# twosigma/Cook

Hardware: AMD Instinct MI355X
Metric: match-cycles/sec at 1M pending x 50k offers (higher is better)
Workload: dtype f64

## Files before the change

cook_amd/csrc/classfit_asm.hpp:

```cpp
#pragma once
#if CF_SLOTS_N == 12
#define CF_O_CTRL "13728"
#define CF_O_CTRL4 "13732"
#define CF_O_ARR "15280"
#define CF_O_CLS32 "9504"
#define CF_SLOT_SHIFT "9"
#define CF_SLOT_N "12"
#define CF_ROW_END "3072"
#elif CF_SLOTS_N == 24
#define CF_O_CTRL "16800"
#define CF_O_CTRL4 "16804"
#define CF_O_ARR "18352"
#define CF_O_CLS32 "12576"
#define CF_SLOT_SHIFT "10"
#define CF_SLOT_N "24"
#define CF_ROW_END "6144"
#else
#error "CF_SLOTS_N: 12 or 24"
#endif
#ifndef CF_ASM_WAIT_READS
#define CF_ASM_WAIT_READS "30"
#endif
#ifdef CF_DELAY_D
#define CF_ASM_DELAY_D "s_sleep 6\n\t"
#else
#define CF_ASM_DELAY_D
#endif
#define CF_ASM_DECIDER_RUN \
   \
  "v_lshl_add_u32 v114, v65, 3, s56\n\t" \
  "ds_read_b64 v[114:115], v114\n\t" \
  "s_ff1_i32_b64 s44, s[42:43]\n\t" \
  "s_lshl_b32 s45, s44, 12\n\t" \
  "s_add_u32 s45, s45, s59\n\t" \
  "s_lshl_b32 s47, s57, 8\n\t" \
  "s_or_b32 s47, s47, s44\n\t" \
  "s_mov_b32 s41, 1\n\t"  \
   \
  "0:\n\t" \
  "v_readlane_b32 s60, v80, s44\n\t" \
  "v_readlane_b32 s61, v81, s44\n\t" \
  "v_readlane_b32 s62, v82, s44\n\t" \
  "s_and_b32 s63, s62, 0xffff00ff\n\t"  \
  "s_cmp_lg_u32 s63, 0\n\t" \
  "s_cbranch_scc1 9f\n\t" \
                                                                                           \
  "v_mov_b32_e32 v88, s47\n\t"                                                                                                          \
  "v_add_u32_e32 v100, s46, v83\n\t"                                                                                                    \
  "s_mov_b64 exec, 1\n\t"                                                                                                               \
  "ds_write_b32 v87, v88 offset:" CF_O_CTRL4 "\n\t"                                                                                              \
  "s_mov_b64 exec, -1\n\t"                                                                                                              \
  "s_mov_b32 s82, " CF_ASM_WAIT_READS "\n\t"              \
  "1:\n\t"                                                                                                                              \
  "ds_read_b32 v92, v100\n\t"                                                                                                           \
  "ds_read_b64 v[94:95], v100 offset:8\n\t"                                                                                             \
  "ds_read_b128 v[96:99], v100 offset:16\n\t"                                                                                           \
  "ds_read_b32 v93, v100\n\t"                                                                                                           \
                                        \
  "v_subrev_u32_e32 v101, s60, v71\n\t"                                                                                                 \
  "v_subrev_u32_e32 v102, s61, v72\n\t"                                                                                                 \
  "v_cvt_f64_u32_e32 v[104:105], v101\n\t"                                                                                              \
  "v_cvt_f64_u32_e32 v[106:107], v102\n\t"                                                                                              \
  "v_mul_f64 v[104:105], v[104:105], v[66:67]\n\t"                                                                                      \
  "v_mul_f64 v[106:107], v[106:107], v[68:69]\n\t"                                                                                      \
  "v_add_f64 v[104:105], v[104:105], v[106:107]\n\t"                                                                                    \
  "v_add_f64 v[104:105], -v[104:105], 1.0\n\t"                                                                                          \
  "v_cmp_le_u32_e64 s[64:65], s60, v71\n\t"                                                                                             \
  "v_cmp_le_u32_e64 s[66:67], s61, v72\n\t"                                                                                             \
  "v_cmp_ne_u32_e64 s[68:69], 0, v64\n\t"                                                                                               \
  "s_and_b64 s[64:65], s[64:65], s[66:67]\n\t"                                                                                          \
  "s_and_b64 s[64:65], s[64:65], s[68:69]\n\t"                                                                                          \
  "s_waitcnt lgkmcnt(0)\n\t"                                                                                                            \
        \
  "s_bfe_u32 s63, s62, 0x4000c\n\t"                                                                                                     \
  "s_cmp_eq_u32 s63, 0\n\t"                                                                                                             \
  "s_cbranch_scc1 3f\n\t"                                                                                                               \
  "v_readlane_b32 s66, v85, s44\n\t"                                                                                                    \
  "v_readlane_b32 s67, v86, s44\n\t"                                                                                                    \
  "s_cmp_lt_u32 s63, 1\n\t"                                                                                                           \
  "s_cbranch_scc1 3f\n\t"                                                                                                               \
  "s_bfe_u32 s72, s66, 0x100000\n\t"                                                                      \
  "s_lshr_b32 s73, s72, 8\n\t"                                                                                                          \
  "s_lshl_b32 s73, s73, 3\n\t"                                                                                                          \
  "s_and_b32 s72, s72, 0xff\n\t"                                                                                                        \
  "v_lshrrev_b64 v[108:109], s73, v[114:115]\n\t"                                                                                       \
  "v_and_b32_e32 v108, 0xff, v108\n\t"                                                                                                  \
  "v_cmp_eq_u32_e64 s[74:75], s72, v108\n\t"                                                                                            \
  "s_and_b64 s[64:65], s[64:65], s[74:75]\n\t"                                                                                          \
  "s_cmp_lt_u32 s63, 2\n\t"                                                                                                           \
  "s_cbranch_scc1 3f\n\t"                                                                                                               \
// ... 15 lines not shown
  "v_and_b32_e32 v108, 0xff, v108\n\t"                                                                                                  \
  "v_cmp_eq_u32_e64 s[74:75], s72, v108\n\t"                                                                                            \
  "s_and_b64 s[64:65], s[64:65], s[74:75]\n\t"                                                                                          \
  "s_cmp_lt_u32 s63, 4\n\t"                                                                                                           \
  "s_cbranch_scc1 3f\n\t"                                                                                                               \
  "s_bfe_u32 s72, s67, 0x100010\n\t"                                                                      \
  "s_lshr_b32 s73, s72, 8\n\t"                                                                                                          \
  "s_lshl_b32 s73, s73, 3\n\t"                                                                                                          \
  "s_and_b32 s72, s72, 0xff\n\t"                                                                                                        \
  "v_lshrrev_b64 v[108:109], s73, v[114:115]\n\t"                                                                                       \
  "v_and_b32_e32 v108, 0xff, v108\n\t"                                                                                                  \
  "v_cmp_eq_u32_e64 s[74:75], s72, v108\n\t"                                                                                            \
  "s_and_b64 s[64:65], s[64:65], s[74:75]\n\t"                                                                                          \
  "3:\n\t"                                                                                                                              \
   \
  "v_and_b32_e32 v108, 0xffffff00, v92\n\t"                                                                                             \
  "v_cmp_eq_u32_e64 s[70:71], s45, v108\n\t"                                                                                            \
  "v_cmp_eq_u32_e64 s[72:73], v92, v93\n\t"                                                                                             \
  "v_sub_u32_e32 v108, v73, v92\n\t"                                                                                                    \
  "v_and_b32_e32 v108, 0xff, v108\n\t"                                                                                                  \
  "v_cmp_gt_u32_e64 s[74:75], 3, v108\n\t"                                                                                              \
  "v_and_b32_e32 v109, 0xffff, v94\n\t"                                                                                                 \
  "v_cmp_ne_u32_e64 s[76:77], v109, v74\n\t"                                                                                            \
  "v_cmp_ne_u32_e64 s[78:79], v109, v75\n\t"                                                                                            \
  "v_cmp_gt_i32_e64 s[80:81], 0, v95\n\t"                                                                                               \
  "s_and_b64 s[74:75], s[74:75], s[76:77]\n\t"                                                                                          \
  "s_and_b64 s[74:75], s[74:75], s[78:79]\n\t"                                                                                          \
  "s_or_b64 s[74:75], s[74:75], s[80:81]\n\t"                                                                                           \
  "s_and_b64 s[72:73], s[70:71], s[72:73]\n\t"                                          \
  "s_and_b64 s[70:71], s[72:73], s[74:75]\n\t"                                                                                            \
  "s_andn2_b64 s[76:77], s[52:53], s[70:71]\n\t"                                                                     \
  "s_cmp_eq_u64 s[76:77], 0\n\t"                                                                                                          \
  "s_cbranch_scc1 2f\n\t"                                                                                                                 \
   \
   \
  "s_and_b64 s[78:79], s[76:77], s[72:73]\n\t"                                                                                            \
  "s_cmp_eq_u64 s[78:79], 0\n\t"                                                                                                          \
  "s_cbranch_scc1 4f\n\t"                                                                                                                 \
  "v_and_b32_e32 v109, 0x3fff, v95\n\t"                                                                                                   \
  "s_and_b64 s[72:73], s[64:65], s[54:55]\n\t"                                                   \
  "10:\n\t"                                                                                                                               \
  "s_ff1_i32_b64 s83, s[78:79]\n\t"                                                                                                       \
  "v_readlane_b32 s63, v109, s83\n\t"                                                                                                     \
  "s_bitset0_b64 s[78:79], s83\n\t"                                                                                                       \
  "v_cmp_eq_u32_e64 vcc, s63, v65\n\t"                                                                                                    \
  "s_and_b64 vcc, vcc, s[72:73]\n\t"                                                                                                      \
  "s_cmp_eq_u64 vcc, 0\n\t"                                                                                                               \
  "s_cbranch_scc1 11f\n\t"                                                                                                                \
  "s_bitset1_b64 s[80:81], s83\n\t"                                                                                                       \
  "s_bitset0_b64 s[76:77], s83\n\t"                                                                                                       \
  "11:\n\t"                                                                                                                               \
  "s_cmp_lg_u64 s[78:79], 0\n\t"                                                                                                          \
  "s_cbranch_scc1 10b\n\t"                                                                                                                \
  "s_cmp_eq_u64 s[76:77], 0\n\t"                                                                                                          \
  "s_cbranch_scc1 2f\n\t"                                                                                                                 \
  "4:\n\t"                                                                                                                                \
  "s_sub_u32 s82, s82, 1\n\t"      \
  "s_cmp_eq_u32 s82, 0\n\t"                                                                                                             \
  "s_cbranch_scc1 9f\n\t"                                                                                                               \
  "s_sleep 1\n\t"                                                                                                                       \
  "s_branch 1b\n\t"                                                                                                                     \
  "2:\n\t"                                                                                                                              \
  "s_andn2_b64 s[74:75], s[52:53], s[80:81]\n\t"                                                                        \
  "s_or_b64 s[64:65], s[64:65], s[74:75]\n\t"                                                          \
  "v_cndmask_b32_e64 v110, v98, v104, s[54:55]\n\t"                                                                                     \
  "v_cndmask_b32_e64 v111, v99, v105, s[54:55]\n\t"                                                                                     \
  "v_cndmask_b32_e64 v110, 0, v110, s[64:65]\n\t"                                                                                       \
  "v_cndmask_b32_e64 v111, 0, v111, s[64:65]\n\t"                                                                                       \
  "v_cvt_f32_f64_e32 v112, v[110:111]\n\t" \
   \
   \
   \
  "s_mov_b64 s[84:85], s[42:43]\n\t" \
  "v_mov_b32_e32 v113, v112\n\t" \
  "s_bitset0_b64 s[84:85], s44\n\t" \
// ... 5 lines not shown
  "s_cmp_eq_u32 s46, " CF_ROW_END "\n\t" \
  "s_cselect_b32 s46, 0, s46\n\t" \
  "v_max_f32_dpp v113, v113, v113 row_half_mirror row_mask:0xf bank_mask:0xf\n\t" \
  "s_lshl_b32 s62, s62, 8\n\t" \
  "s_or_b32 s47, s62, s86\n\t" \
  "v_max_f32_dpp v113, v113, v113 row_mirror row_mask:0xf bank_mask:0xf\n\t" \
  "s_lshl_b32 s63, s86, 12\n\t" \
  "s_add_u32 s45, s59, s63\n\t" \
  "v_max_f32_dpp v113, v113, v113 row_bcast:15 row_mask:0xa bank_mask:0xf\n\t" \
  "v_add_f32_e32 v108, 0x35000000, v112\n\t" \
  "v_and_b32_e32 v109, 0x40000000, v95\n\t" \
  "v_max_f32_dpp v113, v113, v113 row_bcast:31 row_mask:0xc bank_mask:0xf\n\t" \
  "v_cmp_ne_u32_e64 s[70:71], 0, v109\n\t" \
  "s_nop 0\n\t" \
  "v_readlane_b32 s63, v113, 63\n\t" \
  "s_cmp_eq_u32 s63, 0\n\t" \
  "s_cbranch_scc1 8f\n\t"  \
  "v_cmp_eq_f32_e64 s[78:79], s63, v112\n\t" \
  "v_cmp_le_f32_e64 s[76:77], s63, v108\n\t"  \
  "s_and_b64 s[76:77], s[76:77], s[64:65]\n\t"                                      \
  "s_bcnt1_i32_b64 s62, s[76:77]\n\t"                                                                                                   \
  "s_cmp_gt_u32 s62, 1\n\t"                                                                                                             \
  "s_cbranch_scc1 9f\n\t"                                                                                                               \
  "s_and_b64 s[70:71], s[70:71], s[76:77]\n\t"                                                                                          \
  "s_and_b64 s[70:71], s[70:71], s[74:75]\n\t"                       \
  "s_cmp_lg_u64 s[70:71], 0\n\t"                                                                                                        \
  "s_cbranch_scc1 9f\n\t"                                                                                                               \
  "s_ff1_i32_b64 s82, s[78:79]\n\t"                                                                                                     \
  "s_cmp_lt_u32 s82, 58\n\t"                                                                                                            \
  "s_cbranch_scc0 5f\n\t"                                                                                                               \
                                                                                                         \
  "v_readlane_b32 s64, v71, s82\n\t"                                                                                                    \
  "v_readlane_b32 s65, v72, s82\n\t"                                                                                                    \
  "v_readlane_b32 s66, v65, s82\n\t"                                                                                                    \
  "s_sub_u32 s67, s64, s60\n\t"                                                                                                         \
  "s_sub_u32 s70, s65, s61\n\t"                                                                                                         \
  "v_cmp_eq_u32_e64 vcc, s82, v84\n\t"                                                                                                  \
  "v_mov_b32_e32 v88, s67\n\t"                                                                                                          \
  "v_mov_b32_e32 v89, s70\n\t"                                                                                                          \
  "s_cmp_lt_u32 s67, s49\n\t" \
  "s_cselect_b32 s71, 1, 0\n\t" \
  "s_cmp_lt_u32 s70, s50\n\t" \
  "s_cselect_b32 s71, 1, s71\n\t" \
  "v_cndmask_b32_e32 v71, v71, v88, vcc\n\t"                                                                                            \
  "v_cndmask_b32_e32 v72, v72, v89, vcc\n\t"                                                                                            \
  "s_cmp_lg_u32 s71, 0\n\t"                                                                                                             \
  "s_cselect_b64 s[62:63], vcc, 0\n\t"                             \
  "s_mov_b32 s72, s44\n\t"                                                                                                              \
  "s_mov_b32 s73, 0\n\t"                                                                                                                \
  "v_cndmask_b32_e64 v64, v64, 0, s[62:63]\n\t"                                                                                         \
  "s_branch 7f\n\t"                                                                                                                     \
        \
  "5:\n\t"                                                                                                                              \
  "v_readlane_b32 s64, v96, s82\n\t"                                                                                                    \
  "v_readlane_b32 s65, v97, s82\n\t"                                                                                                    \
  "v_readlane_b32 s76, v95, s82\n\t"                                                                                                    \
  "v_readlane_b32 s77, v94, s82\n\t"                                                                                                    \
  "v_readlane_b32 s78, v73, s82\n\t"                                                                                                    \
  "s_sub_u32 s67, s64, s60\n\t"                                                                                                         \
  "s_sub_u32 s70, s65, s61\n\t"                                                                                                         \
  "s_and_b32 s66, s76, 0x3fff\n\t"                                                                                                      \
  "s_bfe_u32 s79, s76, 0x80010\n\t"                                                                                                     \
  "s_and_b32 s73, s77, 0xffff\n\t"                                                                                                      \
  "s_lshr_b32 s81, s77, 16\n\t"                                                                                                         \
  "s_sub_u32 s80, s82, 57\n\t"                                                                                                          \
  "s_cmp_lt_u32 s67, s49\n\t" \
// ... 16 lines not shown
  "v_mov_b32_e32 v100, s78\n\t"                                                                                                         \
  "s_mov_b64 exec, 1\n\t"                                                                                                               \
  "ds_write_b64 v90, v[88:89] offset:" CF_O_ARR "\n\t"                                                                                         \
  "ds_write_b32 v91, v100 offset:" CF_O_CTRL4 "\n\t"                                                                                             \
  "s_mov_b64 exec, -1\n\t"                                                                                                              \
  "v_cmp_eq_u32_e64 vcc, s82, v84\n\t"                                                                                                  \
  "v_mov_b32_e32 v101, s73\n\t" \
  "s_lshl_b32 s62, s80, 8\n\t" \
  "v_cndmask_b32_e32 v75, v75, v74, vcc\n\t" \
  "v_cndmask_b32_e32 v74, v74, v101, vcc\n\t" \
  "v_cndmask_b32_e32 v73, v73, v100, vcc\n\t" \
  "s_lshl_b32 s63, s81, 12\n\t"                                                                                                         \
  "s_or_b32 s72, s44, s62\n\t"                                                                                                          \
  "s_or_b32 s72, s72, s63\n\t"                                                                                                          \
  "s_cmp_lg_u32 s71, 0\n\t"                                                                                                             \
  "s_cbranch_scc1 7f\n\t"                                                                              \
  "s_mul_i32 s62, s79, 56\n\t" \
  "v_add_u32_e32 v90, s62, v87\n\t" \
  "ds_read_b128 v[116:119], v90 offset:" CF_O_CLS32 "\n\t"  \
  "v_mov_b32_e32 v88, s66\n\t" \
  "v_lshl_add_u32 v102, v88, 3, s56\n\t"   \
  "ds_read_b64 v[102:103], v102\n\t"                                                                                        \
  "s_andn2_b64 s[62:63], s[54:55], s[68:69]\n\t"                                                                                        \
  "s_ff1_i32_b64 s83, s[62:63]\n\t"                                                                                                     \
  "v_cmp_eq_u32_e64 vcc, s83, v84\n\t"                                                                                                  \
  "v_mov_b32_e32 v89, s79\n\t"                                                                                                          \
  "v_mov_b32_e32 v91, s67\n\t"                                                                                                          \
  "v_mov_b32_e32 v101, s70\n\t"                                                                                                         \
  "v_cndmask_b32_e64 v64, v64, 1, vcc\n\t"                                                                                              \
  "v_cndmask_b32_e32 v65, v65, v88, vcc\n\t"                                                                                            \
  "v_cndmask_b32_e32 v70, v70, v89, vcc\n\t"                                                                                            \
  "v_cndmask_b32_e32 v71, v71, v91, vcc\n\t"                                                                                            \
  "v_cndmask_b32_e32 v72, v72, v101, vcc\n\t"                                                                                           \
  "s_waitcnt lgkmcnt(0)\n\t"                                                                                                            \
  "v_cndmask_b32_e32 v66, v66, v116, vcc\n\t"                                                                                           \
  "v_cndmask_b32_e32 v67, v67, v117, vcc\n\t"                                                                                           \
  "v_cndmask_b32_e32 v68, v68, v118, vcc\n\t"                                                                                           \
  "v_cndmask_b32_e32 v69, v69, v119, vcc\n\t"  \
  "v_cndmask_b32_e32 v114, v114, v102, vcc\n\t" \
  "v_cndmask_b32_e32 v115, v115, v103, vcc\n\t"                                                                                           \
   \
  "7:\n\t"                                                                                                                              \
  "v_cmp_eq_u32_e64 vcc, s44, v84\n\t"                                                                                                  \
  "v_mov_b32_e32 v88, s66\n\t"                                                                                                          \
  "v_cmp_lt_u32_e64 s[62:63], s67, v80\n\t"                                                                                             \
  "v_cmp_lt_u32_e64 s[76:77], s70, v81\n\t"                                                                                             \
  "v_cndmask_b32_e32 v76, v76, v88, vcc\n\t"                                                                                            \
  "s_or_b64 s[62:63], s[62:63], s[76:77]\n\t"                                                                                           \
  "s_lshl_b64 s[76:77], -2, s44\n\t"                                                                                                    \
  "s_and_b64 s[62:63], s[62:63], s[76:77]\n\t"                                                                                          \
  "s_or_b64 s[38:39], s[38:39], s[62:63]\n\t"                                                                                           \
  "s_min_u32 s37, s37, s67\n\t"                                                                                                         \
  "s_min_u32 s40, s40, s70\n\t"                                                                                                         \
  "s_add_u32 s36, s36, 1\n\t"                                                                                                           \
  "v_mov_b32_e32 v88, s72\n\t"                                                                                                          \
  "v_mov_b32_e32 v89, s73\n\t"                                                                                                          \
  "v_mov_b32_e32 v90, s64\n\t"                                                                                                          \
  "v_mov_b32_e32 v91, s65\n\t" \
  "s_mov_b64 exec, 1\n\t" \
  "ds_write_b128 v77, v[88:91]\n\t" \
  "s_mov_b64 exec, -1\n\t" \
  "v_add_u32_e32 v77, 32, v77\n\t"  \
   \
  "8:\n\t" \
  CF_ASM_DELAY_D \
  "s_mov_b64 s[42:43], s[84:85]\n\t" \
  "s_mov_b32 s44, s86\n\t" \
  "s_add_u32 s57, s57, 1\n\t" \
  "s_cmp_lg_u64 s[42:43], 0\n\t" \
  "s_cbranch_scc1 0b\n\t" \
  "s_mov_b32 s41, 0\n\t" \
  "9:\n\t" \
  "s_waitcnt lgkmcnt(0)\n\t"

#define CF_ASM_CLASS_STEP                                                                                                               \
  "v_mov_b32_e32 v80, s44\n\t"                                                                                                          \
  "s_lshl_b32 s60, s45, 2\n\t"                                                                                                          \
  "s_add_u32 s60, s60, s44\n\t"                                                                                                         \
  "v_mov_b32_e32 v81, s60\n\t"                                                                                                          \
  "ds_read_b64 v[82:83], v80 offset:" CF_O_CTRL "\n\t"                                                                     \
  "ds_read_b32 v84, v81 offset:" CF_O_CTRL4 "\n\t"                                                                   \
  "s_mov_b32 s41, 3\n\t"                                                                                                                \
  "s_waitcnt lgkmcnt(0)\n\t"                                                                                                            \
  "v_readfirstlane_b32 s61, v82\n\t"                                                                                                    \
  "v_readfirstlane_b32 s42, v83\n\t"                                                                                                    \
  "v_readfirstlane_b32 s43, v84\n\t"                                                                                                    \
  "s_cmp_lg_u32 s61, 0\n\t"                                                                                                             \
  "s_cbranch_scc1 9f\n\t"                                                                                                               \
// ... 141 lines not shown
```

cook_amd/csrc/classfit_host.hpp:

```cpp

static int classfit_env() {
  static const int v = [] {
    const char* s = std::getenv("COOK_CLASSFIT");
    return s && (s[0] == '0' || s[0] == '1') ? s[0] - '0' : -1;
  }();
  return v;
}
static bool classfit_by_default(const cook_engine* e) {
  const int f = classfit_env();
  if (f >= 0) return f == 1;
  return g_engines_on_device[e->device & 63].load() >= 6;
}
static size_t cf_lds_bytes_host(unsigned NP, unsigned M, bool eq, unsigned G, unsigned S) {
  size_t n = sizeof(CfFixed) + (size_t)NP * 10u;
  n = (n + 7u) & ~(size_t)7u;
  if (eq) n += (size_t)M * 8u;
  n += ((size_t)G + 1u) * 2u + (size_t)G * 2u + (size_t)S * 2u;
  return n + 64u;
}
bool cf_setup(cook_engine* e, const MatchIn& in, const MatchIn* in_dev, const MatchState& st, const JobRec* jr, const JobCons* jcons, const OfferA* oa, const OfferB* ob,
              CfPoolCtx& ctx) {
  const unsigned K = in.K, M = in.M, G = in.G;
  e->cf_inelig = 0x10000u;
  if (K == 0 || M == 0 || M > CF_SORT_N || G > CF_MAXG || in.good_enough < 1.0 || in.has_x || in.reserved_bits || in.host_dup) return false;
// ... 24 lines not shown
  const unsigned NP = (M + 63u) & ~63u;
  const unsigned S = hc.any_group ? e->cf_group_run_total + hc.n_grouped : 0u;
  if (cf_lds_bytes_host(NP, M, hc.any_eq != 0u, hc.any_group ? G : 0u, S) > CF_LDS_BYTES || S > 60000u) {
    e->cf_inelig = CF_X_SHAPE;
    return false;
  }
  ctx.in = in_dev;
  ctx.st = st;
  ctx.b = b;
  return true;
}
static void cf_prof_print(const uint32_t* q) {
#ifdef CF_PROF
  std::fprintf(stderr, "CFPROF (x16 shader cycles) decider: slow steps %u (candidates %u evaluation %u commit %u) plain steps %u in %u walk-total %u | class wave 1: poll %u answer %u answers %u idle %u idles %u | class wave 2: poll %u answer %u answers %u idle %u idles %u | walk ticks(100MHz) %u | batch boundaries: decider %u, batches without a walked job %u\n", q[27], q[24], q[25], q[26], q[28], q[29], q[31], q[32], q[33], q[35], q[36], q[37], q[40], q[41], q[43], q[44], q[45], q[CFS_TICKS_WALK], q[30], q[38]);
  std::fprintf(stderr, "CFPROF plain steps %u, C++ steps %u; steps that left the plain form: gpu kind %u, novel hosts %u, group %u, answer missing after the re-reads %u, guard band %u, epoch end %u\n", q[46], q[47], q[34] & 65535u, q[34] >> 16, q[39] & 65535u, q[39] >> 16, q[42] & 65535u, q[42] >> 16);
#else
  (void)q;
#endif
}
void cf_run(cook_engine* lead, cook_engine* const* es, unsigned n, hipStream_t stream) {
  cook_engine* e = lead;
  for (unsigned i0 = 0; i0 < n; i0 += (unsigned)CF_PACK) {
    const unsigned c = std::min<unsigned>(CF_PACK, n - i0);
    CfPack pk{};
    for (unsigned x = 0; x < (unsigned)CF_PACK; ++x) pk.c[x] = es[i0 + (x < c ? x : 0u)]->placement.walk;
    KLS("cf_walk", stream, cf_walk, c, CF_THREADS, pk);
  }
  for (unsigned i = 0; i < n; ++i) {
    const CfPoolCtx& c = es[i]->placement.walk;
    const unsigned G = es[i]->last_in.G;
// ... 23 lines not shown
```

cook_amd/csrc/classfit_walk.hpp:

```cpp
#pragma once
#if defined(CF_PROF) && !defined(CF_STATS)
#define CF_STATS 1
#endif
#ifdef CF_STATS
#define CF_STAT(x) x
#define CF_TICKS() cook_ticks()
#else
#define CF_STAT(x) ((void)0)
#define CF_TICKS() 0ull
#endif
#ifdef CF_PROF
#define CF_PROF_T(x) const unsigned long long x = __builtin_readcyclecounter()
#define CF_PROF_ADD(i, d) prof[i] += (unsigned long long)(d)
#define CF_PROF_WHY(n) why = why == 3u ? (n) : why
#define CF_PROF_LEAVE() (why < 4u ? leave_a += 1ull << (16u * why) : leave_b += 1ull << (16u * (why - 4u)))
#else
#define CF_PROF_T(x) ((void)0)
#define CF_PROF_ADD(i, d) ((void)0)
#define CF_PROF_WHY(n) ((void)0)
#define CF_PROF_LEAVE() ((void)0)
#endif

#ifndef CF_AHEAD
#define CF_AHEAD 10
#endif
constexpr unsigned CF_BOARD = CF_AHEAD;
#ifndef CF_SLOTS_N
#define CF_SLOTS_N 12
#endif
constexpr unsigned CF_SLOTS = CF_SLOTS_N;
static_assert(CF_BOARD + 2u <= CF_SLOTS, "a slot is free again before its wave writes it two rows on");
static_assert(CF_SLOTS == 12u || CF_SLOTS == 24u, "cf_slot and classfit_asm.hpp know these two");
static __device__ __forceinline__ unsigned cf_slot(unsigned ord) { return ord - CF_SLOTS * ((ord * 43u) >> (CF_SLOTS == 12u ? 9 : 10)); }
constexpr unsigned CF_OVL = 58;
constexpr unsigned CF_EPOCH_AT = COOK_SHAPE(58, 8);
constexpr unsigned CFW_BOOKS = 4;
enum : unsigned { CFM_EXACT = 1u, CFM_EPOCH = 2u, CFM_BATCH_END = 3u };
enum : unsigned { CFX_NEXT_BASE = 0, CFX_SPARE1, CFX_LOGN, CFX_LOG_APPLIED, CFX_WALK_LO, CFX_WALK_HI, CFX_EX_LANE, CFX_FMAX_LO, CFX_FMAX_HI, CFX_EPOCH, CFX_MATCH_LO, CFX_MATCH_HI,
                  CFX_B1_LO, CFX_B1_HI, CFX_OVN, CFX_MINFC, CFX_MINFM, CFX_N = 24 };
// ... 360 lines not shown
  unsigned minfc_all = wave_uniform_u32(S.envw[CFE_MINFC]), minfm_all = wave_uniform_u32(S.envw[CFE_MINFM]);
  unsigned matched = 0, head = 0;
  unsigned jc = 0, jm = 0, jmeta = 0, jgrp = 0, jeq0 = 0, jeq1 = 0, jnov0 = 0, jnov1 = 0;
  int res = -1;
  unsigned long long b1m = 0ull;
  unsigned seen = 0, gen = 0;
  unsigned tight_applied = 0;
  bool bk_room0 = false, nx_room0 = false, nx_walk = false;
  unsigned st_scans = 0, st_exact = 0, st_open = 0, st_ovwin = 0, st_gpu = 0, st_epochs = 0, st_tight = 0, st_walked = 0, st_dead = 0, st_opendead = 0, st_spins = 0, st_flips = 0,
           st_rewinds = 0;
  unsigned long long tk_epoch = 0, tk_books = 0, tk_walk = 0, tk_phase1 = 0;
#ifdef CF_PROF
  unsigned long long prof[8] = {0, 0, 0, 0, 0, 0, 0, 0}, bnd0 = 0ull;
  unsigned long long leave_a = 0ull, leave_b = 0ull;
#endif
  auto job_of = [&](unsigned s) -> CfJobU {
    CfJobU J;
    J.c = (unsigned)wave_read_lane((int)jc, (int)s), J.m = (unsigned)wave_read_lane((int)jm, (int)s);
    const unsigned meta = (unsigned)wave_read_lane((int)jmeta, (int)s);
    J.kind = meta & 255u, J.L = (meta >> 8) & 15u, J.n_eq = (meta >> 12) & 15u, J.n_nov = (meta >> 16) & 15u, J.grouped = (meta >> 20) & 1u;
    J.grp = 0u, J.eq0 = J.eq1 = 0u, J.nov0 = J.nov1 = 0xFFFFFFFFu;
    if (meta >> 12) {
      J.grp = (unsigned)wave_read_lane((int)jgrp, (int)s), J.eq0 = (unsigned)wave_read_lane((int)jeq0, (int)s), J.eq1 = (unsigned)wave_read_lane((int)jeq1, (int)s),
      J.nov0 = (unsigned)wave_read_lane((int)jnov0, (int)s), J.nov1 = (unsigned)wave_read_lane((int)jnov1, (int)s);
    }
    return J;
  };
  auto tables_room_any = [&](unsigned L, unsigned m) -> bool {
    bool r = S.ovt[L] > m;
    for (unsigned x = 1; x <= (unsigned)CF_CW; ++x) r = r || S.aw[x * CF_LV + L] > m;
// ... 111 lines not shown
          o.hTm = __longlong_as_double((long long)((unsigned long long)ST[5] << 32 | ST[4])), o.cls = ST[6], o.fc = ST[7], o.fm = ST[8], nrm = ST[9], rm1 = ST[10], rm2 = ST[11],
          res = (int)ST[12];
        };
#endif
        while (md == 0u) {
          todo = wave_uniform_u64(todo), cur_ord = wave_uniform_u32(cur_ord), logn = wave_uniform_u32(logn), matched = wave_uniform_u32(matched), gen = wave_uniform_u32(gen);
          minfc_all = wave_uniform_u32(minfc_all), minfm_all = wave_uniform_u32(minfm_all), b1m = wave_uniform_u64(b1m);
#if COOK_HAS_ASM_WALK
          if (todo != 0ull) {
            st_pack();
            CF_PROF_T(f0);
#define CF_U(x) wave_uniform_u32((unsigned)(x))
            cf_u32x8 SC = {CF_U(matched), CF_U(minfc_all), CF_U(b1m), CF_U(b1m >> 32), CF_U(minfm_all), 1u, CF_U(todo), CF_U(todo >> 32)};
            cf_u32x8 AR = {0u, 0u, CF_U(cf_slot(cur_ord) * 8u * (unsigned)sizeof(CfEnt)), 0u, 0u, CF_U(cmin), CF_U(mmin), a_board};
            cf_u32x8 MK = {CF_U(rel0), CF_U(rel0 >> 32), CF_U(ovm), CF_U(ovm >> 32), CF_U(cook_lds_off(S.attr8)), CF_U(cur_ord), 0u, CF_U(base << 12 | (gen & 15u) << 8)};
            asm volatile(CF_ASM_DECIDER_RUN
                         : "+{v[64:79]}"(ST), "+{s[36:43]}"(SC), "+{s[44:51]}"(AR), "+{s[52:59]}"(MK)
                         : "{v[80:87]}"(JB)
                         : "v88", "v89", "v90", "v91", "v92", "v93", "v94", "v95", "v96", "v97", "v98", "v99", "v100", "v101", "v102", "v103", "v104", "v105", "v106", "v107", "v108",
                           "v109", "v110", "v111", "v112", "v113", "v114", "v115", "v116", "v117", "v118", "v119", "s60", "s61", "s62", "s63", "s64", "s65", "s66", "s67", "s68", "s69",
                           "s70", "s71", "s72", "s73", "s74", "s75", "s76", "s77", "s78", "s79", "s80", "s81", "s82", "s83", "s84", "s85", "s86", "vcc", "scc", "memory");
            matched = CF_U(SC[0]), minfc_all = CF_U(SC[1]), minfm_all = CF_U(SC[4]);
            b1m = wave_uniform_u64((unsigned long long)SC[3] << 32 | SC[2]);
            todo = wave_uniform_u64((unsigned long long)SC[7] << 32 | SC[6]);
            logn = (CF_U(ST[13]) - a_log) / (unsigned)sizeof(CfLog);
            CF_PROF_ADD(4, CF_U(MK[5]) - cur_ord);
            cur_ord = CF_U(MK[5]);
#undef CF_U
            CF_PROF_T(f1);
            CF_PROF_ADD(5, f1 - f0);
            WAIT_LDS();
            st_unpack();
          }
#endif
          if (todo == 0ull) {
#ifdef CF_PROF
            bnd0 = __builtin_readcyclecounter();
#endif
            decider_books(logn);
            md = CFM_BATCH_END;
            st_lane0_b32(&S.ctrl[0], md);
// ... 608 lines not shown
      st.summary[2] = st_epochs;
      const unsigned long long t_end = cook_ticks();
      uint32_t* sx = ctl->stats;
      sx[CFS_MATCHED] = matched, sx[CFS_OV_WIN] = st_ovwin, sx[CFS_OPEN] = st_open, sx[CFS_OPEN_DEAD] = st_opendead, sx[CFS_GPU_PLACE] = st_gpu, sx[CFS_EPOCHS] = st_epochs,
      sx[CFS_EXACT] = st_exact, sx[CFS_WALKED] = st_walked, sx[CFS_DEAD_DROP] = st_dead, sx[CFS_BATCHES] = (K + 63u) / 64u, sx[CFS_PRESETTLED] = K - st_walked;
      sx[CFS_TICKS_TOTAL] = (uint32_t)(t_end - t_start), sx[CFS_TICKS_PROLOGUE] = (uint32_t)(t_loop - t_start), sx[CFS_TICKS_EPOCH] = (uint32_t)tk_epoch;
      sx[CFS_TICKS_WALK] = (uint32_t)tk_walk, sx[CFS_TICKS_PHASE1] = (uint32_t)tk_phase1;
      sx[CFS_HWID_DECIDER] = cook_hw_id();
    }
    const unsigned sp = wave_max_u32(!isov ? st_spins : 0u);
    if (lane == 0) ctl->stats[CFS_SPINS] = sp;
  }
  if (is_class_wave && lane == 0) atomicAdd(&ctl->stats[CFS_SCANS], st_scans), atomicAdd(&ctl->stats[CFS_TIGHTEN], st_tight), atomicAdd(&ctl->stats[CFS_REWINDS], st_rewinds);
  if (is_books && lane == 0) ctl->stats[CFS_TICKS_PRECHECK] = (uint32_t)tk_books, ctl->stats[CFS_FLIPS] = st_flips, ctl->stats[CFS_HWID_BOOKS] = cook_hw_id();
#ifdef CF_PROF
  if (lane == 0 && (is_decider || (is_class_wave && lw >= 1u && lw <= 2u && rep == 0u)))
    for (int i = 0; i < 8; ++i)
      if (is_decider || (i != 2 && i != 7 && !(lw == 2u && i == 6))) ctl->stats[24 + 8 * (is_decider ? 0u : lw) + i] = (uint32_t)(prof[i] >> 4);
  if (lane == 0 && is_decider)
    ctl->stats[34] = (uint32_t)leave_a, ctl->stats[39] = (uint32_t)(leave_a >> 32), ctl->stats[42] = (uint32_t)leave_b, ctl->stats[46] = (uint32_t)prof[4], ctl->stats[47] = (uint32_t)prof[3];
#endif
#undef n_cls
#undef n_kind
#undef NP
}

static __device__ __forceinline__ void cf_walk_pool(char* lds, const MatchIn* __restrict__ inp, const MatchState& st, const CfBuf& b) {
  const unsigned tid = threadIdx.x, lane = lane_id(), w = wave_id();
  CfCtl* ctl = b.ctl;
  const unsigned K = inp->K, M = ctl->M, G = inp->G;
  const unsigned NP = (M + 63u) & ~63u;
  const unsigned long long t_start = cook_ticks();
  const bool any_eq = ctl->any_eq != 0u, any_group = ctl->any_group != 0u;
// ... 80 lines not shown
    }
  }
  for (unsigned x = tid; x < ctl->n_cls; x += CF_THREADS) S.cls[x] = ctl->cls[x];
  for (unsigned x = tid; x < CFX_N; x += CF_THREADS) S.misc[x] = 0u;
  for (unsigned x = tid; x < 8u * CF_LV; x += CF_THREADS) S.pw[x] = 0u, S.aw[x] = 0u;
  for (unsigned x = tid; x < 8u; x += CF_THREADS) S.ctrl[x] = 0u;
  for (unsigned x = tid; x < CF_MAXKIND * CF_LV; x += CF_THREADS) S.gk[x] = 0u;
  for (unsigned x = tid; x < (unsigned)CF_LV; x += CF_THREADS) S.ovt[x] = 0u;
  for (unsigned x = tid; x < CF_SLOTS * 8u; x += CF_THREADS) S.board[x].tag = 0xFFFFFFFFu;
  __syncthreads();
  if (w == 0u) {
    cf_walk_role<0>(S, st, b, 0u, 0u, 1u, t_start);
  } else if (w == CFW_BOOKS) {
    cf_walk_role<2>(S, st, b, 0u, 0u, 1u, t_start);
  } else {
    const unsigned p = w < CFW_BOOKS ? w - 1u : w - 2u, np = (unsigned)CF_WAVES - 2u;
    unsigned used = 0, zsets = 0;
    for (unsigned ci = 0; ci < ctl->n_cls; ++ci) {
      const unsigned g = S.cls[ci].wave;
      used |= 1u << g;
      if (S.cls[ci].kind == 0u) zsets |= 1u << g;
    }
    used = wave_uniform_u32(used), zsets = wave_uniform_u32(zsets);
    unsigned myset = 0, rep = 0, nrep = 0, k = 0;
    for (unsigned pass = 0; pass < np && k < np; ++pass) {
      const unsigned from = pass == 0u ? used : (zsets ? zsets : used);
      if (from == 0u) break;
      for (unsigned g = 1; g <= (unsigned)CF_CW && k < np; ++g)
        if ((from >> g) & 1u) {
          if (k == p) myset = g;
          ++k;
// ... 25 lines not shown
```

Measured before the change: 23.28.

## Hoist row reads and job lanes out of decider loop, interleave compares

Restructures the decider's inline-asm loop so the first job's lane reads and the row's LDS reads are issued before the loop head. The SALU/VALU compares are interleaved with the f64 arithmetic so they can hide the LDS wait. Re-read trips now reissue the row reads explicitly, and the loop exit path is reworked. It also adds optional variants (early row prefetch, an alternate SIMD0 wave mapping) and a segment-profiling build, all off by default.

Measured after the change: 23.36, median of 6. No clear change (+0.4%).

```diff
diff --git a/cook_amd/csrc/classfit_asm.hpp b/cook_amd/csrc/classfit_asm.hpp
--- a/cook_amd/csrc/classfit_asm.hpp
+++ b/cook_amd/csrc/classfit_asm.hpp
@@ -26,54 +26,102 @@
 #else
 #define CF_ASM_DELAY_D
 #endif
+#define CF_ASM_ROW_READS                      \
+  "ds_read_b32 v92, v100\n\t"                 \
+  "ds_read_b64 v[94:95], v100 offset:8\n\t"   \
+  "ds_read_b128 v[96:99], v100 offset:16\n\t" \
+  "ds_read_b32 v93, v100\n\t"
+#ifndef CF_EARLY_ROW
+#define CF_EARLY_ROW 0
+#endif
+#if CF_EARLY_ROW
+#define CF_ASM_NEXT_ROW              \
+  "v_add_u32_e32 v100, s46, v83\n\t" \
+  CF_ASM_ROW_READS                   \
+  CF_ASM_T0
+#define CF_ASM_FIRST_ROW CF_ASM_NEXT_ROW
+#define CF_ASM_ROW_AT_HEAD
+#else
+#define CF_ASM_NEXT_ROW
+#define CF_ASM_FIRST_ROW
+#define CF_ASM_ROW_AT_HEAD           \
+  "v_add_u32_e32 v100, s46, v83\n\t" \
+  CF_ASM_ROW_READS                   \
+  CF_ASM_T0
+#endif
+#define CF_ASM_NEXT_JOB              \
+  "v_readlane_b32 s60, v80, s86\n\t" \
+  "v_readlane_b32 s61, v81, s86\n\t" \
+  "v_readlane_b32 s62, v82, s86\n\t"
+#ifdef CF_PROF_SEG
+#define CF_ASM_T_INIT "s_mov_b32 s92, 0\n\ts_mov_b32 s94, 0\n\t"
+#define CF_ASM_T0 "s_memtime s[88:89]\n\t"
+#define CF_ASM_T1 "s_memtime s[90:91]\n\ts_waitcnt lgkmcnt(0)\n\ts_sub_u32 s95, s94, s92\n\ts_add_u32 s98, s98, s95\n\ts_mov_b32 s94, s92\n\ts_cmp_eq_u32 s63, 0\n\t"
+#define CF_ASM_T2                                                                                                                                     \
+  "s_memtime s[92:93]\n\ts_waitcnt lgkmcnt(0)\n\ts_sub_u32 s95, s90, s88\n\ts_add_u32 s96, s96, s95\n\ts_sub_u32 s95, s92, s90\n\ts_add_u32 s97, s97, s95\n\t" \
+  "s_add_u32 s99, s99, 1\n\ts_mov_b32 s94, s92\n\t"
+#define CF_ASM_T3 "s_memtime s[94:95]\n\t"
+#define CF_ASM_T_EXIT "s_sub_u32 s95, s94, s92\n\ts_add_u32 s98, s98, s95\n\t"
+#define CF_ASM_COUNT_REREAD "s_cmp_eq_u32 s82, " CF_ASM_WAIT_READS "\n\ts_cselect_b32 s83, 0x10001, 1\n\ts_add_u32 s41, s41, s83\n\t"
+#define CF_ASM_STATUS(n)
+#else
+#define CF_ASM_T_INIT
+#define CF_ASM_T0
+#define CF_ASM_T1
+#define CF_ASM_T2
+#define CF_ASM_T3
+#define CF_ASM_T_EXIT
+#define CF_ASM_COUNT_REREAD
+#define CF_ASM_STATUS(n) "s_mov_b32 s41, " n "\n\t"
+#endif
 #define CF_ASM_DECIDER_RUN \
+   \
    \
   "v_lshl_add_u32 v114, v65, 3, s56\n\t" \
   "ds_read_b64 v[114:115], v114\n\t" \
   "s_ff1_i32_b64 s44, s[42:43]\n\t" \
   "s_lshl_b32 s45, s44, 12\n\t" \
+  "v_readlane_b32 s60, v80, s44\n\t" \
+  "v_readlane_b32 s61, v81, s44\n\t" \
+  "v_readlane_b32 s62, v82, s44\n\t" \
   "s_add_u32 s45, s45, s59\n\t" \
   "s_lshl_b32 s47, s57, 8\n\t" \
   "s_or_b32 s47, s47, s44\n\t" \
-  "s_mov_b32 s41, 1\n\t"  \
-   \
-  "0:\n\t" \
-  "v_readlane_b32 s60, v80, s44\n\t" \
-  "v_readlane_b32 s61, v81, s44\n\t" \
-  "v_readlane_b32 s62, v82, s44\n\t" \
+  CF_ASM_STATUS("1")  \
+  CF_ASM_T_INIT \
   "s_and_b32 s63, s62, 0xffff00ff\n\t"  \
   "s_cmp_lg_u32 s63, 0\n\t" \
   "s_cbranch_scc1 9f\n\t" \
-                                                                                           \
+  CF_ASM_FIRST_ROW \
+   \
+  "0:\n\t" \
+                                                                                                                    \
   "v_mov_b32_e32 v88, s47\n\t"                                                                                                          \
-  "v_add_u32_e32 v100, s46, v83\n\t"                                                                                                    \
   "s_mov_b64 exec, 1\n\t"                                                                                                               \
   "ds_write_b32 v87, v88 offset:" CF_O_CTRL4 "\n\t"                                                                                              \
   "s_mov_b64 exec, -1\n\t"                                                                                                              \
+  CF_ASM_ROW_AT_HEAD                                                                                                                    \
   "s_mov_b32 s82, " CF_ASM_WAIT_READS "\n\t"              \
   "1:\n\t"                                                                                                                              \
-  "ds_read_b32 v92, v100\n\t"                                                                                                           \
-  "ds_read_b64 v[94:95], v100 offset:8\n\t"                                                                                             \
-  "ds_read_b128 v[96:99], v100 offset:16\n\t"                                                                                           \
-  "ds_read_b32 v93, v100\n\t"                                                                                                           \
-                                        \
+   \
   "v_subrev_u32_e32 v101, s60, v71\n\t"                                                                                                 \
   "v_subrev_u32_e32 v102, s61, v72\n\t"                                                                                                 \
+  "v_cmp_le_u32_e64 s[64:65], s60, v71\n\t"                                                                                             \
   "v_cvt_f64_u32_e32 v[104:105], v101\n\t"                                                                                              \
   "v_cvt_f64_u32_e32 v[106:107], v102\n\t"                                                                                              \
+  "v_cmp_le_u32_e64 s[66:67], s61, v72\n\t"                                                                                             \
   "v_mul_f64 v[104:105], v[104:105], v[66:67]\n\t"                                                                                      \
   "v_mul_f64 v[106:107], v[106:107], v[68:69]\n\t"                                                                                      \
+  "v_cmp_ne_u32_e64 s[68:69], 0, v64\n\t"                                                                                               \
+  "s_bfe_u32 s63, s62, 0x4000c\n\t"                                                                    \
   "v_add_f64 v[104:105], v[104:105], v[106:107]\n\t"                                                                                    \
+  "s_and_b64 s[64:65], s[64:65], s[66:67]\n\t"                                                                                          \
   "v_add_f64 v[104:105], -v[104:105], 1.0\n\t"                                                                                          \
-  "v_cmp_le_u32_e64 s[64:65], s60, v71\n\t"                                                                                             \
-  "v_cmp_le_u32_e64 s[66:67], s61, v72\n\t"                                                                                             \
-  "v_cmp_ne_u32_e64 s[68:69], 0, v64\n\t"                                                                                               \
-  "s_and_b64 s[64:65], s[64:65], s[66:67]\n\t"                                                                                          \
   "s_and_b64 s[64:65], s[64:65], s[68:69]\n\t"                                                                                          \
-  "s_waitcnt lgkmcnt(0)\n\t"                                                                                                            \
+  "s_cmp_eq_u32 s63, 0\n\t"                                                                                                             \
+  "s_waitcnt lgkmcnt(0)\n\t"                                                                                  \
+  CF_ASM_T1                                                                                                                             \
         \
-  "s_bfe_u32 s63, s62, 0x4000c\n\t"                                                                                                     \
-  "s_cmp_eq_u32 s63, 0\n\t"                                                                                                             \
   "s_cbranch_scc1 3f\n\t"                                                                                                               \
   "v_readlane_b32 s66, v85, s44\n\t"                                                                                                    \
   "v_readlane_b32 s67, v86, s44\n\t"                                                                                                    \
@@ -119,20 +167,21 @@
   "s_and_b64 s[64:65], s[64:65], s[74:75]\n\t"                                                                                          \
   "3:\n\t"                                                                                                                              \
    \
+                     \
   "v_and_b32_e32 v108, 0xffffff00, v92\n\t"                                                                                             \
+  "v_sub_u32_e32 v110, v73, v92\n\t"                                                                                                    \
+  "v_and_b32_e32 v109, 0xffff, v94\n\t"                                                                                                 \
+  "v_cmp_eq_u32_e64 s[72:73], v92, v93\n\t"                                                                                             \
   "v_cmp_eq_u32_e64 s[70:71], s45, v108\n\t"                                                                                            \
-  "v_cmp_eq_u32_e64 s[72:73], v92, v93\n\t"                                                                                             \
-  "v_sub_u32_e32 v108, v73, v92\n\t"                                                                                                    \
-  "v_and_b32_e32 v108, 0xff, v108\n\t"                                                                                                  \
-  "v_cmp_gt_u32_e64 s[74:75], 3, v108\n\t"                                                                                              \
-  "v_and_b32_e32 v109, 0xffff, v94\n\t"                                                                                                 \
+  "v_and_b32_e32 v110, 0xff, v110\n\t"                                                                                                  \
   "v_cmp_ne_u32_e64 s[76:77], v109, v74\n\t"                                                                                            \
   "v_cmp_ne_u32_e64 s[78:79], v109, v75\n\t"                                                                                            \
+  "v_cmp_gt_u32_e64 s[74:75], 3, v110\n\t"                                                                                              \
   "v_cmp_gt_i32_e64 s[80:81], 0, v95\n\t"                                                                                               \
+  "s_and_b64 s[72:73], s[70:71], s[72:73]\n\t"                                          \
+  "s_and_b64 s[76:77], s[76:77], s[78:79]\n\t"                                                                                          \
   "s_and_b64 s[74:75], s[74:75], s[76:77]\n\t"                                                                                          \
-  "s_and_b64 s[74:75], s[74:75], s[78:79]\n\t"                                                                                          \
   "s_or_b64 s[74:75], s[74:75], s[80:81]\n\t"                                                                                           \
-  "s_and_b64 s[72:73], s[70:71], s[72:73]\n\t"                                          \
   "s_and_b64 s[70:71], s[72:73], s[74:75]\n\t"                                                                                            \
   "s_andn2_b64 s[76:77], s[52:53], s[70:71]\n\t"                                                                     \
   "s_cmp_eq_u64 s[76:77], 0\n\t"                                                                                                          \
@@ -160,10 +209,12 @@
   "s_cmp_eq_u64 s[76:77], 0\n\t"                                                                                                          \
   "s_cbranch_scc1 2f\n\t"                                                                                                                 \
   "4:\n\t"                                                                                                                                \
+  CF_ASM_COUNT_REREAD                                                                                                                   \
   "s_sub_u32 s82, s82, 1\n\t"      \
   "s_cmp_eq_u32 s82, 0\n\t"                                                                                                             \
   "s_cbranch_scc1 9f\n\t"                                                                                                               \
   "s_sleep 1\n\t"                                                                                                                       \
+  CF_ASM_ROW_READS                                                                                \
   "s_branch 1b\n\t"                                                                                                                     \
   "2:\n\t"                                                                                                                              \
   "s_andn2_b64 s[74:75], s[52:53], s[80:81]\n\t"                                                                        \
@@ -199,42 +250,50 @@
   "v_cmp_ne_u32_e64 s[70:71], 0, v109\n\t" \
   "s_nop 0\n\t" \
   "v_readlane_b32 s63, v113, 63\n\t" \
+  CF_ASM_T2 \
+  "s_and_b64 s[70:71], s[70:71], s[74:75]\n\t"  \
   "s_cmp_eq_u32 s63, 0\n\t" \
-  "s_cbranch_scc1 8f\n\t"  \
+  "s_cbranch_scc1 12f\n\t"  \
+  "v_cmp_le_f32_e64 s[76:77], s63, v108\n\t"  \
   "v_cmp_eq_f32_e64 s[78:79], s63, v112\n\t" \
-  "v_cmp_le_f32_e64 s[76:77], s63, v108\n\t"  \
   "s_and_b64 s[76:77], s[76:77], s[64:65]\n\t"                                      \
+  "s_ff1_i32_b64 s82, s[78:79]\n\t"           \
   "s_bcnt1_i32_b64 s62, s[76:77]\n\t"                                                                                                   \
+  "s_and_b64 s[70:71], s[70:71], s[76:77]\n\t"                       \
   "s_cmp_gt_u32 s62, 1\n\t"                                                                                                             \
   "s_cbranch_scc1 9f\n\t"                                                                                                               \
-  "s_and_b64 s[70:71], s[70:71], s[76:77]\n\t"                                                                                          \
-  "s_and_b64 s[70:71], s[70:71], s[74:75]\n\t"                       \
   "s_cmp_lg_u64 s[70:71], 0\n\t"                                                                                                        \
   "s_cbranch_scc1 9f\n\t"                                                                                                               \
-  "s_ff1_i32_b64 s82, s[78:79]\n\t"                                                                                                     \
   "s_cmp_lt_u32 s82, 58\n\t"                                                                                                            \
   "s_cbranch_scc0 5f\n\t"                                                                                                               \
                                                                                                          \
   "v_readlane_b32 s64, v71, s82\n\t"                                                                                                    \
   "v_readlane_b32 s65, v72, s82\n\t"                                                                                                    \
   "v_readlane_b32 s66, v65, s82\n\t"                                                                                                    \
+  CF_ASM_NEXT_ROW                                                                                                                       \
+  "v_cmp_eq_u32_e64 vcc, s82, v84\n\t"                                                                                               \
   "s_sub_u32 s67, s64, s60\n\t"                                                                                                         \
   "s_sub_u32 s70, s65, s61\n\t"                                                                                                         \
-  "v_cmp_eq_u32_e64 vcc, s82, v84\n\t"                                                                                                  \
-  "v_mov_b32_e32 v88, s67\n\t"                                                                                                          \
-  "v_mov_b32_e32 v89, s70\n\t"                                                                                                          \
+  "s_mov_b32 s72, s44\n\t"                                                                                                              \
+  "s_mov_b32 s73, 0\n\t"                                                                                                                \
   "s_cmp_lt_u32 s67, s49\n\t" \
   "s_cselect_b32 s71, 1, 0\n\t" \
   "s_cmp_lt_u32 s70, s50\n\t" \
   "s_cselect_b32 s71, 1, s71\n\t" \
+  "v_mov_b32_e32 v88, s67\n\t"                                                                                                          \
+  "v_mov_b32_e32 v89, s70\n\t"                                                                                                          \
+  "s_cmp_lg_u32 s71, 0\n\t"                                                                                                             \
+  "s_cselect_b64 s[62:63], vcc, 0\n\t"                             \
   "v_cndmask_b32_e32 v71, v71, v88, vcc\n\t"                                                                                            \
   "v_cndmask_b32_e32 v72, v72, v89, vcc\n\t"                                                                                            \
-  "s_cmp_lg_u32 s71, 0\n\t"                                                                                                             \
-  "s_cselect_b64 s[62:63], vcc, 0\n\t"                             \
-  "s_mov_b32 s72, s44\n\t"                                                                                                              \
-  "s_mov_b32 s73, 0\n\t"                                                                                                                \
   "v_cndmask_b32_e64 v64, v64, 0, s[62:63]\n\t"                                                                                         \
   "s_branch 7f\n\t"                                                                                                                     \
+                                                          \
+  "12:\n\t"                                                                                                                             \
+  CF_ASM_NEXT_ROW                                                                                                                       \
+  CF_ASM_NEXT_JOB                                                                                                                       \
+  "s_and_b32 s63, s62, 0xffff00ff\n\t"                                                                                                \
+  "s_branch 8f\n\t"                                                                                                                     \
         \
   "5:\n\t"                                                                                                                              \
   "v_readlane_b32 s64, v96, s82\n\t"                                                                                                    \
@@ -281,7 +340,7 @@
   "s_or_b32 s72, s44, s62\n\t"                                                                                                          \
   "s_or_b32 s72, s72, s63\n\t"                                                                                                          \
   "s_cmp_lg_u32 s71, 0\n\t"                                                                                                             \
-  "s_cbranch_scc1 7f\n\t"                                                                              \
+  "s_cbranch_scc1 13f\n\t"                                                                             \
   "s_mul_i32 s62, s79, 56\n\t" \
   "v_add_u32_e32 v90, s62, v87\n\t" \
   "ds_read_b128 v[116:119], v90 offset:" CF_O_CLS32 "\n\t"  \
@@ -306,27 +365,34 @@
   "v_cndmask_b32_e32 v69, v69, v119, vcc\n\t"  \
   "v_cndmask_b32_e32 v114, v114, v102, vcc\n\t" \
   "v_cndmask_b32_e32 v115, v115, v103, vcc\n\t"                                                                                           \
+                       \
+  "13:\n\t"                                                                                                                             \
+  CF_ASM_NEXT_ROW                                                                                                                       \
+   \
    \
   "7:\n\t"                                                                                                                              \
+  CF_ASM_NEXT_JOB                                                                                                                       \
   "v_cmp_eq_u32_e64 vcc, s44, v84\n\t"                                                                                                  \
+  "v_cmp_lt_u32_e64 s[74:75], s67, v80\n\t"                                                                                             \
+  "v_cmp_lt_u32_e64 s[76:77], s70, v81\n\t"                                                                                             \
   "v_mov_b32_e32 v88, s66\n\t"                                                                                                          \
-  "v_cmp_lt_u32_e64 s[62:63], s67, v80\n\t"                                                                                             \
-  "v_cmp_lt_u32_e64 s[76:77], s70, v81\n\t"                                                                                             \
+  "s_lshl_b64 s[78:79], -2, s44\n\t"                                                                                                    \
+  "s_and_b32 s63, s62, 0xffff00ff\n\t"                                \
   "v_cndmask_b32_e32 v76, v76, v88, vcc\n\t"                                                                                            \
-  "s_or_b64 s[62:63], s[62:63], s[76:77]\n\t"                                                                                           \
-  "s_lshl_b64 s[76:77], -2, s44\n\t"                                                                                                    \
-  "s_and_b64 s[62:63], s[62:63], s[76:77]\n\t"                                                                                          \
-  "s_or_b64 s[38:39], s[38:39], s[62:63]\n\t"                                                                                           \
+  "s_or_b64 s[74:75], s[74:75], s[76:77]\n\t"                                                                                           \
+  "v_mov_b32_e32 v88, s72\n\t"                                                                                                          \
+  "s_and_b64 s[74:75], s[74:75], s[78:79]\n\t"                                                                                          \
+  "v_mov_b32_e32 v89, s73\n\t"                                                                                                          \
+  "s_or_b64 s[38:39], s[38:39], s[74:75]\n\t"                                                                                           \
+  "v_mov_b32_e32 v90, s64\n\t"                                                                                                          \
   "s_min_u32 s37, s37, s67\n\t"                                                                                                         \
+  "v_mov_b32_e32 v91, s65\n\t" \
   "s_min_u32 s40, s40, s70\n\t"                                                                                                         \
   "s_add_u32 s36, s36, 1\n\t"                                                                                                           \
-  "v_mov_b32_e32 v88, s72\n\t"                                                                                                          \
-  "v_mov_b32_e32 v89, s73\n\t"                                                                                                          \
-  "v_mov_b32_e32 v90, s64\n\t"                                                                                                          \
-  "v_mov_b32_e32 v91, s65\n\t" \
   "s_mov_b64 exec, 1\n\t" \
   "ds_write_b128 v77, v[88:91]\n\t" \
   "s_mov_b64 exec, -1\n\t" \
+  CF_ASM_T3 \
   "v_add_u32_e32 v77, 32, v77\n\t"  \
    \
   "8:\n\t" \
@@ -334,11 +400,16 @@
   "s_mov_b64 s[42:43], s[84:85]\n\t" \
   "s_mov_b32 s44, s86\n\t" \
   "s_add_u32 s57, s57, 1\n\t" \
-  "s_cmp_lg_u64 s[42:43], 0\n\t" \
+  "s_cmp_eq_u64 s[42:43], 0\n\t" \
+  "s_cbranch_scc1 14f\n\t" \
+  "s_cmp_eq_u32 s63, 0\n\t" \
   "s_cbranch_scc1 0b\n\t" \
-  "s_mov_b32 s41, 0\n\t" \
+  "s_branch 9f\n\t" \
+  "14:\n\t" \
+  CF_ASM_STATUS("0") \
   "9:\n\t" \
-  "s_waitcnt lgkmcnt(0)\n\t"
+  "s_waitcnt lgkmcnt(0)\n\t"  \
+  CF_ASM_T_EXIT
 
 #define CF_ASM_CLASS_STEP                                                                                                               \
   "v_mov_b32_e32 v80, s44\n\t"                                                                                                          \
diff --git a/cook_amd/csrc/classfit_host.hpp b/cook_amd/csrc/classfit_host.hpp
--- a/cook_amd/csrc/classfit_host.hpp
+++ b/cook_amd/csrc/classfit_host.hpp
@@ -62,6 +62,9 @@
 #ifdef CF_PROF
   std::fprintf(stderr, "CFPROF (x16 shader cycles) decider: slow steps %u (candidates %u evaluation %u commit %u) plain steps %u in %u walk-total %u | class wave 1: poll %u answer %u answers %u idle %u idles %u | class wave 2: poll %u answer %u answers %u idle %u idles %u | walk ticks(100MHz) %u | batch boundaries: decider %u, batches without a walked job %u\n", q[27], q[24], q[25], q[26], q[28], q[29], q[31], q[32], q[33], q[35], q[36], q[37], q[40], q[41], q[43], q[44], q[45], q[CFS_TICKS_WALK], q[30], q[38]);
   std::fprintf(stderr, "CFPROF plain steps %u, C++ steps %u; steps that left the plain form: gpu kind %u, novel hosts %u, group %u, answer missing after the re-reads %u, guard band %u, epoch end %u\n", q[46], q[47], q[34] & 65535u, q[34] >> 16, q[39] & 65535u, q[39] >> 16, q[42] & 65535u, q[42] >> 16);
+#ifdef CF_PROF_SEG
+  std::fprintf(stderr, "CFPROF plain steps stamped %u: (x16 shader cycles) row's reads issued -> behind the wait %u, -> behind the maximum %u, -> behind the log store %u; re-read trips %u, steps that re-read %u\n", q[44], q[40], q[41], q[43], q[45], q[37]);
+#endif
 #else
   (void)q;
 #endif
diff --git a/cook_amd/csrc/classfit_walk.hpp b/cook_amd/csrc/classfit_walk.hpp
--- a/cook_amd/csrc/classfit_walk.hpp
+++ b/cook_amd/csrc/classfit_walk.hpp
@@ -1,6 +1,14 @@
 #pragma once
 #if defined(CF_PROF) && !defined(CF_STATS)
 #define CF_STATS 1
+#endif
+#ifdef CF_PROF_SEG
+#ifndef CF_PROF
+#error "CF_PROF_SEG is a variant of the CF_PROF build: define both"
+#endif
+#define CF_SEG_BUILD 1
+#else
+#define CF_SEG_BUILD 0
 #endif
 #ifdef CF_STATS
 #define CF_STAT(x) x
@@ -23,6 +31,9 @@
 
 #ifndef CF_AHEAD
 #define CF_AHEAD 10
+#endif
+#ifndef CF_SIMD0_MAP
+#define CF_SIMD0_MAP 0
 #endif
 constexpr unsigned CF_BOARD = CF_AHEAD;
 #ifndef CF_SLOTS_N
@@ -413,6 +424,9 @@
   unsigned long long prof[8] = {0, 0, 0, 0, 0, 0, 0, 0}, bnd0 = 0ull;
   unsigned long long leave_a = 0ull, leave_b = 0ull;
 #endif
+#ifdef CF_PROF_SEG
+  unsigned long long seg[6] = {0, 0, 0, 0, 0, 0};
+#endif
   auto job_of = [&](unsigned s) -> CfJobU {
     CfJobU J;
     J.c = (unsigned)wave_read_lane((int)jc, (int)s), J.m = (unsigned)wave_read_lane((int)jm, (int)s);
@@ -554,10 +568,19 @@
             cf_u32x8 SC = {CF_U(matched), CF_U(minfc_all), CF_U(b1m), CF_U(b1m >> 32), CF_U(minfm_all), 1u, CF_U(todo), CF_U(todo >> 32)};
             cf_u32x8 AR = {0u, 0u, CF_U(cf_slot(cur_ord) * 8u * (unsigned)sizeof(CfEnt)), 0u, 0u, CF_U(cmin), CF_U(mmin), a_board};
             cf_u32x8 MK = {CF_U(rel0), CF_U(rel0 >> 32), CF_U(ovm), CF_U(ovm >> 32), CF_U(cook_lds_off(S.attr8)), CF_U(cur_ord), 0u, CF_U(base << 12 | (gen & 15u) << 8)};
+#ifdef CF_PROF_SEG
+            SC[5] = 0u;
+            cf_u32x4 PS = {0u, 0u, 0u, 0u};
+#define CF_SEG_OUT , "+{s[96:99]}"(PS)
+#define CF_SEG_CLOBBER "s88", "s89", "s90", "s91", "s92", "s93", "s94", "s95",
+#else
+#define CF_SEG_OUT
+#define CF_SEG_CLOBBER
+#endif
             asm volatile(CF_ASM_DECIDER_RUN
-                         : "+{v[64:79]}"(ST), "+{s[36:43]}"(SC), "+{s[44:51]}"(AR), "+{s[52:59]}"(MK)
+                         : "+{v[64:79]}"(ST), "+{s[36:43]}"(SC), "+{s[44:51]}"(AR), "+{s[52:59]}"(MK) CF_SEG_OUT
                          : "{v[80:87]}"(JB)
-                         : "v88", "v89", "v90", "v91", "v92", "v93", "v94", "v95", "v96", "v97", "v98", "v99", "v100", "v101", "v102", "v103", "v104", "v105", "v106", "v107", "v108",
+                         : CF_SEG_CLOBBER "v88", "v89", "v90", "v91", "v92", "v93", "v94", "v95", "v96", "v97", "v98", "v99", "v100", "v101", "v102", "v103", "v104", "v105", "v106", "v107", "v108",
                            "v109", "v110", "v111", "v112", "v113", "v114", "v115", "v116", "v117", "v118", "v119", "s60", "s61", "s62", "s63", "s64", "s65", "s66", "s67", "s68", "s69",
                            "s70", "s71", "s72", "s73", "s74", "s75", "s76", "s77", "s78", "s79", "s80", "s81", "s82", "s83", "s84", "s85", "s86", "vcc", "scc", "memory");
             matched = CF_U(SC[0]), minfc_all = CF_U(SC[1]), minfm_all = CF_U(SC[4]);
@@ -565,6 +588,9 @@
             todo = wave_uniform_u64((unsigned long long)SC[7] << 32 | SC[6]);
             logn = (CF_U(ST[13]) - a_log) / (unsigned)sizeof(CfLog);
             CF_PROF_ADD(4, CF_U(MK[5]) - cur_ord);
+#ifdef CF_PROF_SEG
+            seg[0] += CF_U(PS[0]), seg[1] += CF_U(PS[1]), seg[2] += CF_U(PS[2]), seg[3] += CF_U(PS[3]), seg[4] += CF_U(SC[5]) & 65535u, seg[5] += CF_U(SC[5]) >> 16;
+#endif
             cur_ord = CF_U(MK[5]);
 #undef CF_U
             CF_PROF_T(f1);
@@ -1203,9 +1229,16 @@
   if (is_class_wave && lane == 0) atomicAdd(&ctl->stats[CFS_SCANS], st_scans), atomicAdd(&ctl->stats[CFS_TIGHTEN], st_tight), atomicAdd(&ctl->stats[CFS_REWINDS], st_rewinds);
   if (is_books && lane == 0) ctl->stats[CFS_TICKS_PRECHECK] = (uint32_t)tk_books, ctl->stats[CFS_FLIPS] = st_flips, ctl->stats[CFS_HWID_BOOKS] = cook_hw_id();
 #ifdef CF_PROF
+#ifdef CF_PROF_SEG
+  if (lane == 0 && is_decider)
+    ctl->stats[40] = (uint32_t)(seg[0] >> 4), ctl->stats[41] = (uint32_t)(seg[1] >> 4), ctl->stats[43] = (uint32_t)(seg[2] >> 4), ctl->stats[44] = (uint32_t)seg[3], ctl->stats[45] = (uint32_t)seg[4],
+    ctl->stats[37] = (uint32_t)seg[5];
+  if (lane == 0 && (is_decider || (is_class_wave && lw == 1u && rep == 0u)))
+#else
   if (lane == 0 && (is_decider || (is_class_wave && lw >= 1u && lw <= 2u && rep == 0u)))
+#endif
     for (int i = 0; i < 8; ++i)
-      if (is_decider || (i != 2 && i != 7 && !(lw == 2u && i == 6))) ctl->stats[24 + 8 * (is_decider ? 0u : lw) + i] = (uint32_t)(prof[i] >> 4);
+      if (is_decider || (i != 2 && i != 7 && !(lw == 2u && i == 6) && !(CF_SEG_BUILD && i == 5))) ctl->stats[24 + 8 * (is_decider ? 0u : lw) + i] = (uint32_t)(prof[i] >> 4);
   if (lane == 0 && is_decider)
     ctl->stats[34] = (uint32_t)leave_a, ctl->stats[39] = (uint32_t)(leave_a >> 32), ctl->stats[42] = (uint32_t)leave_b, ctl->stats[46] = (uint32_t)prof[4], ctl->stats[47] = (uint32_t)prof[3];
 #endif
@@ -1316,7 +1349,13 @@
   } else if (w == CFW_BOOKS) {
     cf_walk_role<2>(S, st, b, 0u, 0u, 1u, t_start);
   } else {
+#if CF_SIMD0_MAP == 0
     const unsigned p = w < CFW_BOOKS ? w - 1u : w - 2u, np = (unsigned)CF_WAVES - 2u;
+#else
+    constexpr unsigned n0 = (unsigned)CF_WAVES / 4u - 2u;
+    const unsigned np = (unsigned)CF_WAVES - 2u - (CF_SIMD0_MAP == 2 ? n0 : 0u);
+    const unsigned p = (w & 3u) != 0u ? w - 1u - w / 4u : (unsigned)CF_WAVES - 2u - n0 + (w / 4u - 2u);
+#endif
     unsigned used = 0, zsets = 0;
     for (unsigned ci = 0; ci < ctl->n_cls; ++ci) {
       const unsigned g = S.cls[ci].wave;
```
